# instadeepai/InstaGeo-E2E-Geospatial-ML

Hardware: AMD Instinct MI355X
Metric: HLS chips/sec (train fwd+bwd+AdamW), prithvi_eo_v1_100 224x224x6 T=1 (higher is better)
Workload: dtype bf16; 1 GPU; BASELINE.json configs[1]: Prithvi-100M fine-tune, Sen1Floods11-shaped synthetic int16 chips (6 bands, T=1, 224x224, 2 classes, weights [1,3], ignore -1, dropout 0.1); per_gpu_batch=432, global_batch=432, parallelism=dp1, launch=eager, deterministic=True

## Files before the change

instageo-e2e-geospatial-ml_amd/csrc/attention2.hip:

```cpp
#include <stdlib.h>

#include "common.h"

#ifdef IG_A2_PROF
__device__ unsigned long long g_a2prof[8 * 48];
#define A2P_INIT_X const bool a2p_on = blockIdx.x == 0 && blockIdx.y == 1 && blockIdx.z == 1 && (threadIdx.x & 63) == 0;
#define A2P_MARK(I) { if (a2p_on) g_a2prof[(threadIdx.x >> 6) * 48 + (I)] = __builtin_readcyclecounter(); }
#define A2P_MARKV(I, V) { float a2p_v = (V); asm volatile("" ::"v"(a2p_v)); if (a2p_on) g_a2prof[(threadIdx.x >> 6) * 48 + (I)] = __builtin_readcyclecounter(); }
extern "C" int ig_debug_a2prof(unsigned long long* dst) { return hipMemcpyFromSymbol(dst, HIP_SYMBOL(g_a2prof), sizeof(g_a2prof)) == hipSuccess ? 0 : -1; }
#else
#define A2P_INIT_X
#define A2P_MARK(I)
#define A2P_MARKV(I, V)
#endif

namespace {

constexpr int A2_WAVES = 7, A2_THREADS = 448, A2_QB = 224, A2_CH = 224;
constexpr int A2_TILE = A2_CH * 128;
typedef __attribute__((ext_vector_type(16))) float f32x16;
typedef __attribute__((ext_vector_type(8))) short s16x8;
typedef __attribute__((address_space(3))) s16x4* lds_s16x4;
typedef __attribute__((address_space(3))) char* lds_char_ptr;

__device__ __forceinline__ void glds16(const void* gsrc, unsigned lds_dst) {
    unsigned keep;
    lds_dst = __builtin_amdgcn_readfirstlane(lds_dst);
    asm volatile("s_mov_b32 %0, m0\n\ts_mov_b32 m0, %2\n\ts_nop 0\n\tglobal_load_lds_dwordx4 %1, off\n\ts_mov_b32 m0, %0"
                 : "=&s"(keep)
                 : "v"(gsrc), "s"(lds_dst)
                 : "memory");
}
__device__ __forceinline__ int k_swz(int row) { return (row >> 1) & 7; }
__device__ __forceinline__ int v_swz(int row) { return ((row >> 1) & 1) << 2; }

__device__ __forceinline__ f32x16 mfma32(bf16x8_t a, bf16x8_t b, f32x16 c) { return __builtin_amdgcn_mfma_f32_32x32x16_bf16(a, b, c, 0, 0, 0); }
template <bool SPLIT>
__device__ __forceinline__ f32x16 mma3(bf16x8_t ah, bf16x8_t al, bf16x8_t bh, bf16x8_t bl, f32x16 c) {
    c = mfma32(ah, bh, c);
    if constexpr (SPLIT) {
        c = mfma32(ah, bl, c);
        c = mfma32(al, bh, c);
    }
    return c;
}

template <bool SPLIT>
__device__ __forceinline__ void a2_store_row64(bf16_t* hi, bf16_t* lo, size_t orow, const f32x16 (&acc)[2], float scale, int lh) {
#pragma unroll
    for (int dh = 0; dh < 2; ++dh)
#pragma unroll
        for (int gp = 0; gp < 2; ++gp) {
            float va[4], vc[4];
#pragma unroll
            for (int e = 0; e < 4; ++e) va[e] = acc[dh][8 * gp + e] * scale, vc[e] = acc[dh][8 * gp + 4 + e] * scale;
            const uint32_t a0 = pack_bf2(va[0], va[1]), a1 = pack_bf2(va[2], va[3]), c0 = pack_bf2(vc[0], vc[1]), c1 = pack_bf2(vc[2], vc[3]);
            {
                const auto s0 = __builtin_amdgcn_permlane32_swap(a0, c0, false, false);
                const auto s1 = __builtin_amdgcn_permlane32_swap(a1, c1, false, false);
                *reinterpret_cast<uint4*>(hi + orow + 32 * dh + 16 * gp + 8 * lh) = lh == 0 ? make_uint4(a0, a1, s0[1], s1[1]) : make_uint4(s0[0], s1[0], c0, c1);
            }
            if constexpr (SPLIT) {
                const uint32_t la0 = pack_bf2(va[0] - __uint_as_float(a0 << 16), va[1] - __uint_as_float(a0 & 0xffff0000u));
                const uint32_t la1 = pack_bf2(va[2] - __uint_as_float(a1 << 16), va[3] - __uint_as_float(a1 & 0xffff0000u));
                const uint32_t lc0 = pack_bf2(vc[0] - __uint_as_float(c0 << 16), vc[1] - __uint_as_float(c0 & 0xffff0000u));
                const uint32_t lc1 = pack_bf2(vc[2] - __uint_as_float(c1 << 16), vc[3] - __uint_as_float(c1 & 0xffff0000u));
                const auto s0 = __builtin_amdgcn_permlane32_swap(la0, lc0, false, false);
                const auto s1 = __builtin_amdgcn_permlane32_swap(la1, lc1, false, false);
                *reinterpret_cast<uint4*>(lo + orow + 32 * dh + 16 * gp + 8 * lh) = lh == 0 ? make_uint4(la0, la1, s0[1], s1[1]) : make_uint4(s0[0], s1[0], lc0, lc1);
            }
        }
}

template <bool SPLIT>
__global__ __launch_bounds__(A2_THREADS) void attn2_fwd_kernel(const bf16_t* __restrict__ qkv_hi, const bf16_t* __restrict__ qkv_lo,
                                                               bf16_t* __restrict__ out_hi, bf16_t* __restrict__ out_lo,
                                                               float* __restrict__ lse, int N, int H, float scale) {
    extern __shared__ __attribute__((aligned(16))) char smem[];
    char* k_hi = smem;
    char* v_hi = smem + A2_TILE;
    char* k_lo = smem + 2 * A2_TILE;
    char* v_lo = smem + 3 * A2_TILE;
    const int tid = threadIdx.x, lane = tid & 63;
    const int wave = __builtin_amdgcn_readfirstlane(tid >> 6);
    const int lr = lane & 31, lh = lane >> 5;
    const int h = blockIdx.y, b = blockIdx.z;
    const long RS = 3L * H * 64;
    const bf16_t* base_hi = qkv_hi + (long)b * N * RS + h * 64;
    const bf16_t* base_lo = SPLIT ? qkv_lo + (long)b * N * RS + h * 64 : nullptr;
    const int q0 = blockIdx.x * A2_QB + wave * 32;
    const bool active = q0 < N;

    bf16x8_t qh[4], ql[4];
    {
        const int qr = min(q0 + lr, N - 1);
#pragma unroll
        for (int s = 0; s < 4; ++s) {
            qh[s] = __builtin_bit_cast(bf16x8_t, *reinterpret_cast<const uint4*>(base_hi + (long)qr * RS + 16 * s + 8 * lh));
            if constexpr (SPLIT) ql[s] = __builtin_bit_cast(bf16x8_t, *reinterpret_cast<const uint4*>(base_lo + (long)qr * RS + 16 * s + 8 * lh));
            else ql[s] = qh[s];
        }
    }
    f32x16 o[2];
#pragma unroll
    for (int i = 0; i < 2; ++i)
#pragma unroll
        for (int r = 0; r < 16; ++r) o[i][r] = 0.f;
    float m_run = -INFINITY, l_run = 0.f;
    const float c2 = scale * 1.44269504088896340736f;
    const unsigned lds_base = (unsigned)(uintptr_t)(lds_char_ptr)smem;

    for (int c0 = 0; c0 < N; c0 += A2_CH) {
        if (c0 > 0) __syncthreads();
#pragma unroll
        for (int i = 0; i < 4; ++i) {
            const int row = (wave * 4 + i) * 8 + (lane >> 3);
            const int key = min(c0 + row, N - 1);
            const long goff = (long)key * RS;
            const int ck = ((lane & 7) ^ k_swz(row)) * 8, cv = ((lane & 7) ^ v_swz(row)) * 8;
            const unsigned dst = lds_base + (wave * 4 + i) * 1024;
            glds16(base_hi + goff + H * 64 + ck, dst);
            glds16(base_hi + goff + 2 * H * 64 + cv, dst + A2_TILE);
            if constexpr (SPLIT) {
                glds16(base_lo + goff + H * 64 + ck, dst + 2 * A2_TILE);
                glds16(base_lo + goff + 2 * H * 64 + cv, dst + 3 * A2_TILE);
            }
        }
        asm volatile("s_waitcnt vmcnt(0)" ::: "memory");
        __syncthreads();
        if (!active) continue;
        const int ntile = min(A2_CH / 32, (N - c0 + 31) >> 5);
#define A2_QK(KT, DST)                                                                                       \
    {                                                                                                        \
        _Pragma("unroll") for (int r_ = 0; r_ < 16; ++r_) DST[r_] = 0.f;                                     \
        const int krow_ = (KT)*32 + lr;                                                                      \
        _Pragma("unroll") for (int s_ = 0; s_ < 4; ++s_) {                                                   \
            const int off_ = krow_ * 128 + (((2 * s_ + lh) ^ k_swz(krow_)) << 4);                            \
            const bf16x8_t kh_ = *reinterpret_cast<const bf16x8_t*>(k_hi + off_);                            \
            const bf16x8_t kl_ = SPLIT ? *reinterpret_cast<const bf16x8_t*>(k_lo + off_) : kh_;              \
            DST = mma3<SPLIT>(kh_, kl_, qh[s_], ql[s_], DST);                                                \
        }                                                                                                    \
    }
        f32x16 st_next;
        A2_QK(0, st_next)
        for (int kt = 0; kt < ntile; ++kt) {
            f32x16 st = st_next;
            if (kt + 1 < ntile) A2_QK(kt + 1, st_next)
            const int key0 = c0 + kt * 32;
            if (key0 + 32 > N) {
                asm volatile("" ::: "memory");
#pragma unroll
                for (int r = 0; r < 16; ++r)
                    if (key0 + 8 * (r >> 2) + 4 * lh + (r & 3) >= N) st[r] = -INFINITY;
            }
            float mx = st[0];
#pragma unroll
            for (int r = 1; r < 16; ++r) mx = fmaxf(mx, st[r]);
            {
                const auto sw = __builtin_amdgcn_permlane32_swap(__float_as_uint(mx), __float_as_uint(mx), false, false);
                mx = fmaxf(__uint_as_float(sw[0]), __uint_as_float(sw[1]));
            }
            const float m_tile = mx * c2;
            if (__builtin_amdgcn_ballot_w64(m_tile > m_run + 8.0f) != 0) {
                const float m_new = fmaxf(m_run, m_tile);
                const float alpha = __builtin_amdgcn_exp2f(m_run - m_new);
#pragma unroll
                for (int i = 0; i < 2; ++i)
// ... 234 lines not shown
#pragma unroll
        for (int o = 16; o >= 1; o >>= 1) {
            const bool up = (lr & o) != 0;
#pragma unroll
            for (int i = 0; i < o; ++i) {
                const float snd = up ? v[i] : v[i + o], kp = up ? v[i + o] : v[i];
                v[i] = kp + __shfl_xor(snd, o, 64);
            }
        }
        scr[(wave * 2 + 0) * 64 + 32 * (lr >> 4) + 8 * ((lr >> 2) & 3) + 4 * lh + (lr & 3)] = v[0];
    }
    {
        float v[32];
#pragma unroll
        for (int s = 0; s < 4; ++s)
#pragma unroll
            for (int e = 0; e < 8; ++e) {
                const float dv = SPLIT ? (float)dh[s][e] + (float)dl[s][e] : (float)dh[s][e];
                v[s * 8 + e] = valid ? dv : 0.f;
            }
#pragma unroll
        for (int o = 16; o >= 1; o >>= 1) {
            const bool up = (lr & o) != 0;
#pragma unroll
            for (int i = 0; i < o; ++i) {
                const float snd = up ? v[i] : v[i + o], kp = up ? v[i + o] : v[i];
                v[i] = kp + __shfl_xor(snd, o, 64);
            }
        }
        scr[(wave * 2 + 1) * 64 + 16 * (lr >> 3) + 8 * lh + (lr & 7)] = v[0];
    }
    __syncthreads();
    if (tid < 128) {
        const int part = tid >> 6, col = tid & 63;
        float t = 0.f;
#pragma unroll
        for (int w = 0; w < A2_WAVES; ++w) t += scr[(w * 2 + part) * 64 + col];
        ig_red_add(dbias + (size_t)(part * 2) * H * 64 + h * 64 + col, t);
    }
}

template <bool SPLIT>
__global__ __launch_bounds__(A2_THREADS) void attn2_bwd_dkv_kernel(const bf16_t* __restrict__ qkv_hi, const bf16_t* __restrict__ qkv_lo,
                                                                   const bf16_t* __restrict__ do_hi, const bf16_t* __restrict__ do_lo,
                                                                   const float* __restrict__ lse, const float* __restrict__ delta,
                                                                   bf16_t* __restrict__ dqkv_hi, bf16_t* __restrict__ dqkv_lo, int N, int H,
                                                                   float scale) {
    extern __shared__ __attribute__((aligned(16))) char smem[];
    char* q_hi = smem;
    char* d_hi = smem + A2_TILE;
    char* q_lo = smem + 2 * A2_TILE;
    char* d_lo = smem + 3 * A2_TILE;
    float* s_lse = reinterpret_cast<float*>(smem + (SPLIT ? 4 : 2) * A2_TILE);
    float* s_del = s_lse + A2_CH;
    const int tid = threadIdx.x, lane = tid & 63;
    const int wave = __builtin_amdgcn_readfirstlane(tid >> 6);
    const int lr = lane & 31, lh = lane >> 5;
    const int h = blockIdx.y, b = blockIdx.z;
    const long RS = 3L * H * 64, OS = (long)H * 64;
    const bf16_t* base_hi = qkv_hi + (long)b * N * RS + h * 64;
    const bf16_t* base_lo = SPLIT ? qkv_lo + (long)b * N * RS + h * 64 : nullptr;
    const bf16_t* dob_hi = do_hi + (long)b * N * OS + h * 64;
    const bf16_t* dob_lo = SPLIT ? do_lo + (long)b * N * OS + h * 64 : nullptr;
    const int k0 = blockIdx.x * A2_QB + wave * 32;
    const bool active = k0 < N;
    const int key = k0 + lr, kr = min(key, N - 1);

    bf16x8_t kh[4], kl[4], vh[4], vl[4];
#pragma unroll
    for (int s = 0; s < 4; ++s) {
        kh[s] = own_frag(base_hi + H * 64, RS, kr, s, lh);
        vh[s] = own_frag(base_hi + 2 * H * 64, RS, kr, s, lh);
        kl[s] = SPLIT ? own_frag(base_lo + H * 64, RS, kr, s, lh) : kh[s];
        vl[s] = SPLIT ? own_frag(base_lo + 2 * H * 64, RS, kr, s, lh) : vh[s];
    }
    const float c2 = scale * 1.44269504088896340736f;
    f32x16 dk[2], dv[2];
#pragma unroll
    for (int i = 0; i < 2; ++i)
#pragma unroll
        for (int r = 0; r < 16; ++r) dk[i][r] = 0.f, dv[i][r] = 0.f;
    const unsigned lds_base = (unsigned)(uintptr_t)(lds_char_ptr)smem;

    for (int c0 = 0; c0 < N; c0 += A2_CH) {
        if (c0 > 0) __syncthreads();
        dma_image(lds_base, base_hi, RS, c0, N, wave, lane);
        dma_image(lds_base + A2_TILE, dob_hi, OS, c0, N, wave, lane);
        if constexpr (SPLIT) {
            dma_image(lds_base + 2 * A2_TILE, base_lo, RS, c0, N, wave, lane);
            dma_image(lds_base + 3 * A2_TILE, dob_lo, OS, c0, N, wave, lane);
        }
        if (tid < A2_CH) {
            const int qq = c0 + tid;
            s_lse[tid] = qq < N ? lse[((long)b * H + h) * N + qq] * 1.44269504088896340736f : INFINITY;
            s_del[tid] = qq < N ? delta[((long)b * H + h) * N + qq] : 0.f;
        }
        asm volatile("s_waitcnt vmcnt(0)" ::: "memory");
        __syncthreads();
        if (!active) continue;
        const int ntile = min(A2_CH / 32, (N - c0 + 31) >> 5);
        for (int qt = 0; qt < ntile; ++qt) {
            f32x16 st, dp;
#pragma unroll
            for (int r = 0; r < 16; ++r) st[r] = 0.f, dp[r] = 0.f;
#pragma unroll
            for (int s = 0; s < 4; ++s) {
                const bf16x8_t ah = rows_frag(q_hi, qt * 32, s, lr, lh);
                const bf16x8_t al = SPLIT ? rows_frag(q_lo, qt * 32, s, lr, lh) : ah;
                st = mma3<SPLIT>(ah, al, kh[s], kl[s], st);
            }
#pragma unroll
            for (int s = 0; s < 4; ++s) {
                const bf16x8_t ah = rows_frag(d_hi, qt * 32, s, lr, lh);
                const bf16x8_t al = SPLIT ? rows_frag(d_lo, qt * 32, s, lr, lh) : ah;
                dp = mma3<SPLIT>(ah, al, vh[s], vl[s], dp);
            }
            f32x16 ds;
#pragma unroll
            for (int g = 0; g < 4; ++g) {
                const float4 l4 = *reinterpret_cast<const float4*>(s_lse + qt * 32 + 8 * g + 4 * lh);
                const float4 d4 = *reinterpret_cast<const float4*>(s_del + qt * 32 + 8 * g + 4 * lh);
                const float ll[4] = {l4.x, l4.y, l4.z, l4.w}, dd[4] = {d4.x, d4.y, d4.z, d4.w};
#pragma unroll
                for (int e = 0; e < 4; ++e) {
                    const float pv = __builtin_amdgcn_exp2f(fmaf(st[4 * g + e], c2, -ll[e]));
                    st[4 * g + e] = pv;
                    ds[4 * g + e] = pv * (dp[4 * g + e] - dd[e]);
                }
            }
#pragma unroll
            for (int s = 0; s < 2; ++s) {
                bf16x8_t ph, pl, sh, sl;
                pack_step<SPLIT>(st, s, ph, pl);
                pack_step<SPLIT>(ds, s, sh, sl);
#pragma unroll
                for (int dhf = 0; dhf < 2; ++dhf) {
                    const bf16x8_t th = tr_frag(d_hi, qt * 32, s, 32 * dhf, lane);
                    const bf16x8_t tl = SPLIT ? tr_frag(d_lo, qt * 32, s, 32 * dhf, lane) : th;
                    dv[dhf] = mma3<SPLIT>(th, tl, ph, pl, dv[dhf]);
                    const bf16x8_t uh = tr_frag(q_hi, qt * 32, s, 32 * dhf, lane);
                    const bf16x8_t ul = SPLIT ? tr_frag(q_lo, qt * 32, s, 32 * dhf, lane) : uh;
                    dk[dhf] = mma3<SPLIT>(uh, ul, sh, sl, dk[dhf]);
                }
            }
        }
    }
    if (!active || key >= N) return;
    const size_t orow = ((size_t)b * N + key) * RS + h * 64;
    a2_store_row64<SPLIT>(dqkv_hi, dqkv_lo, orow + (size_t)H * 64, dk, scale, lh);
    a2_store_row64<SPLIT>(dqkv_hi, dqkv_lo, orow + 2 * (size_t)H * 64, dv, 1.f, lh);
}


constexpr int A2F_DQP = 68;
constexpr int A2F_SLAB = 32 * 72;
constexpr int A2F_OFF_K = 2 * A2_TILE;
constexpr int A2F_OFF_DQ = 2 * A2_TILE;
constexpr int A2F_OFF_SLAB = A2F_OFF_DQ + A2_CH * A2F_DQP * 4;
constexpr int A2F_OFF_LSE = A2F_OFF_SLAB + A2_WAVES * A2F_SLAB;
constexpr int A2F_SMEM = A2F_OFF_LSE + 2 * A2_CH * 4;

__device__ __forceinline__ bf16x8_t tr_slab(const char* slab, int s, int lane) {
    const int g16 = lane >> 4, i16 = lane & 15;
    const int r0 = 16 * s + 4 * (g16 >> 1) + (i16 >> 2), r1 = r0 + 8;
    const int cb = (16 * (g16 & 1) + 4 * (i16 & 3)) * 2;
    const s16x4 a0 = __builtin_amdgcn_ds_read_tr16_b64_v4i16((lds_s16x4)(slab + r0 * 72 + cb));
    const s16x4 a1 = __builtin_amdgcn_ds_read_tr16_b64_v4i16((lds_s16x4)(slab + r1 * 72 + cb));
    const s16x8 av = {a0[0], a0[1], a0[2], a0[3], a1[0], a1[1], a1[2], a1[3]};
    return __builtin_bit_cast(bf16x8_t, av);
}

__global__ __launch_bounds__(A2_THREADS) void attn2_bwd_fused_kernel(const bf16_t* __restrict__ qkv_hi, const bf16_t* __restrict__ do_hi,
                                                                     const bf16_t* __restrict__ o_hi, const float* __restrict__ lse,
                                                                     float* __restrict__ delta, bf16_t* __restrict__ dqkv_hi, int N, int H,
                                                                     float scale, float* __restrict__ dbias) {
    extern __shared__ __attribute__((aligned(16))) char smem[];
    A2P_INIT_X
    char* q_img = smem;
    char* d_img = smem + A2_TILE;
    char* k_img = smem + A2F_OFF_K;
    float* s_dq = reinterpret_cast<float*>(smem + A2F_OFF_DQ);
    float* s_lse = reinterpret_cast<float*>(smem + A2F_OFF_LSE);
    float* s_del = s_lse + A2_CH;
    const int tid = threadIdx.x, lane = tid & 63;
    const int wave = __builtin_amdgcn_readfirstlane(tid >> 6);
    char* slab = smem + A2F_OFF_SLAB + wave * A2F_SLAB;
    const int lr = lane & 31, lh = lane >> 5;
    const long RS = 3L * H * 64, OS = (long)H * 64;
    const int h = blockIdx.y, b = blockIdx.z;
    const bf16_t* base = qkv_hi + (long)b * N * RS + h * 64;
    const bf16_t* dob = do_hi + (long)b * N * OS + h * 64;
    const bf16_t* ob = o_hi + (long)b * N * OS + h * 64;
    const int k0 = wave * 32;
    const bool active = k0 < N;
    const int key = k0 + lr, kr = min(key, N - 1);
    const unsigned lds_base = (unsigned)(uintptr_t)(lds_char_ptr)smem;

    dma_image(lds_base, base, RS, 0, N, wave, lane);
    dma_image(lds_base + A2_TILE, dob, OS, 0, N, wave, lane);
    dma_image(lds_base + A2F_OFF_K, base + H * 64, RS, 0, N, wave, lane);
    bf16x8_t kh[4], vh[4];
#pragma unroll
    for (int s = 0; s < 4; ++s) {
        kh[s] = own_frag(base + H * 64, RS, kr, s, lh);
        vh[s] = own_frag(base + 2 * H * 64, RS, kr, s, lh);
    }
    {
        float dl = 0.f;
#pragma unroll
        for (int s = 0; s < 4; ++s) {
            const bf16x8_t oh = own_frag(ob, OS, kr, s, lh), dh = own_frag(dob, OS, kr, s, lh);
#pragma unroll
            for (int e = 0; e < 8; ++e) dl = fmaf((float)oh[e], (float)dh[e], dl);
        }
        const auto sw = __builtin_amdgcn_permlane32_swap(__float_as_uint(dl), __float_as_uint(dl), false, false);
        dl = __uint_as_float(sw[0]) + __uint_as_float(sw[1]);
        if (lh == 0) {
            if (key < N) delta[((long)b * H + h) * N + key] = dl;
            s_lse[key] = key < N ? lse[((long)b * H + h) * N + key] * 1.44269504088896340736f : INFINITY;
            s_del[key] = key < N ? dl : 0.f;
        }
    }
    const float c2 = scale * 1.44269504088896340736f;
    const float kmask = key < N ? 1.f : 0.f;
    f32x16 dk[2], dv[2];
#pragma unroll
    for (int i = 0; i < 2; ++i)
#pragma unroll
        for (int r = 0; r < 16; ++r) dk[i][r] = 0.f, dv[i][r] = 0.f;
    A2P_MARK(0)
    asm volatile("s_waitcnt vmcnt(0)" ::: "memory");
    A2P_MARK(1)
    __syncthreads();
    A2P_MARK(2)
    const int ntile = (N + 31) >> 5;
    bf16x8_t kt[2][2];
#pragma unroll
    for (int s = 0; s < 2; ++s)
#pragma unroll
        for (int dhf = 0; dhf < 2; ++dhf) kt[s][dhf] = tr_frag(k_img, k0, s, 32 * dhf, lane);
    asm volatile("s_waitcnt lgkmcnt(0)" ::: "memory");
    __syncthreads();
    A2P_MARK(3)
    for (int step = 0; step < A2_WAVES; ++step) {
        const int qt = (wave + step) % A2_WAVES;
        A2P_MARK(4 + step * 6)
        if (active && qt < ntile) {
            f32x16 st, dp;
#pragma unroll
            for (int r = 0; r < 16; ++r) st[r] = 0.f, dp[r] = 0.f;
#pragma unroll
            for (int s = 0; s < 4; ++s) st = mfma32(rows_frag(q_img, qt * 32, s, lr, lh), kh[s], st);
#pragma unroll
            for (int s = 0; s < 4; ++s) dp = mfma32(rows_frag(d_img, qt * 32, s, lr, lh), vh[s], dp);
            bf16x8_t tdo[2][2], tq[2][2];
#pragma unroll
            for (int s = 0; s < 2; ++s)
#pragma unroll
                for (int dhf = 0; dhf < 2; ++dhf) {
                    tdo[s][dhf] = tr_frag(d_img, qt * 32, s, 32 * dhf, lane);
                    tq[s][dhf] = tr_frag(q_img, qt * 32, s, 32 * dhf, lane);
                }
            A2P_MARKV(5 + step * 6, st[0] + dp[0])
            f32x16 ds;
#pragma unroll
            for (int g = 0; g < 4; ++g) {
                const float4 l4 = *reinterpret_cast<const float4*>(s_lse + qt * 32 + 8 * g + 4 * lh);
                const float4 d4 = *reinterpret_cast<const float4*>(s_del + qt * 32 + 8 * g + 4 * lh);
                const float ll[4] = {l4.x, l4.y, l4.z, l4.w}, dd[4] = {d4.x, d4.y, d4.z, d4.w};
#pragma unroll
                for (int e = 0; e < 4; ++e) {
                    const float pv = __builtin_amdgcn_exp2f(fmaf(st[4 * g + e], c2, -ll[e])) * kmask;
                    st[4 * g + e] = pv;
                    ds[4 * g + e] = pv * (dp[4 * g + e] - dd[e]);
                }
            }
            A2P_MARKV(6 + step * 6, ds[0] + ds[15])
#pragma unroll
            for (int s = 0; s < 2; ++s) {
                bf16x8_t ph, pl, sh, sl;
                pack_step<false>(st, s, ph, pl);
                pack_step<false>(ds, s, sh, sl);
                const uint4 su = __builtin_bit_cast(uint4, sh);
                *reinterpret_cast<uint2*>(slab + lr * 72 + (16 * s + 4 * lh) * 2) = make_uint2(su.x, su.y);
                *reinterpret_cast<uint2*>(slab + lr * 72 + (16 * s + 8 + 4 * lh) * 2) = make_uint2(su.z, su.w);
#pragma unroll
                for (int dhf = 0; dhf < 2; ++dhf) {
                    dv[dhf] = mfma32(tdo[s][dhf], ph, dv[dhf]);
                    dk[dhf] = mfma32(tq[s][dhf], sh, dk[dhf]);
                }
            }
            A2P_MARKV(7 + step * 6, dv[0][0] + dk[0][0] + dv[1][15] + dk[1][15])
            asm volatile("s_waitcnt lgkmcnt(0)" ::: "memory");
            f32x16 dq0, dq1;
            {
                const float* row = s_dq + (qt * 32 + lr) * A2F_DQP + 4 * lh;
#pragma unroll
                for (int g = 0; g < 4; ++g) {
                    float4 o0 = make_float4(0.f, 0.f, 0.f, 0.f), o1 = o0;
                    if (step > 0) o0 = *reinterpret_cast<const float4*>(row + 8 * g), o1 = *reinterpret_cast<const float4*>(row + 32 + 8 * g);
                    dq0[4 * g] = o0.x, dq0[4 * g + 1] = o0.y, dq0[4 * g + 2] = o0.z, dq0[4 * g + 3] = o0.w;
                    dq1[4 * g] = o1.x, dq1[4 * g + 1] = o1.y, dq1[4 * g + 2] = o1.z, dq1[4 * g + 3] = o1.w;
                }
            }
            const bf16x8_t b0 = tr_slab(slab, 0, lane), b1 = tr_slab(slab, 1, lane);
            dq0 = mfma32(kt[0][0], b0, dq0);
            dq1 = mfma32(kt[0][1], b0, dq1);
            dq0 = mfma32(kt[1][0], b1, dq0);
            dq1 = mfma32(kt[1][1], b1, dq1);
            {
                float* row = s_dq + (qt * 32 + lr) * A2F_DQP + 4 * lh;
#pragma unroll
                for (int g = 0; g < 4; ++g) {
                    *reinterpret_cast<float4*>(row + 8 * g) = make_float4(dq0[4 * g], dq0[4 * g + 1], dq0[4 * g + 2], dq0[4 * g + 3]);
                    *reinterpret_cast<float4*>(row + 32 + 8 * g) = make_float4(dq1[4 * g], dq1[4 * g + 1], dq1[4 * g + 2], dq1[4 * g + 3]);
                }
            }
            A2P_MARK(8 + step * 6)
        }
        __syncthreads();
        A2P_MARK(9 + step * 6)
    }
    float cbq[8] = {0.f, 0.f, 0.f, 0.f, 0.f, 0.f, 0.f, 0.f}, cbv[8] = {0.f, 0.f, 0.f, 0.f, 0.f, 0.f, 0.f, 0.f};
    for (int it = tid; it < N * 8; it += A2_THREADS) {
        const int q = it >> 3, c = it & 7;
        const float4 v0 = *reinterpret_cast<const float4*>(s_dq + q * A2F_DQP + 8 * c), v1 = *reinterpret_cast<const float4*>(s_dq + q * A2F_DQP + 8 * c + 4);
        const float f[8] = {v0.x * scale, v0.y * scale, v0.z * scale, v0.w * scale, v1.x * scale, v1.y * scale, v1.z * scale, v1.w * scale};
        *reinterpret_cast<uint4*>(dqkv_hi + ((size_t)b * N + q) * RS + h * 64 + 8 * c) = pack8(f);
#pragma unroll
        for (int e = 0; e < 8; ++e) cbq[e] += f[e];
    }
    A2P_MARK(46)
    if (dbias) {
        for (int it = tid; it < N * 8; it += A2_THREADS) {
            const int q = it >> 3, c = it & 7;
            float f[8];
            unpack8(*reinterpret_cast<const uint4*>(d_img + q * 128 + ((c ^ sw2(q)) << 4)), f);
#pragma unroll
            for (int e = 0; e < 8; ++e) cbv[e] += f[e];
        }
        A2P_MARKV(40, cbv[0] + cbv[7])
        float* scr = reinterpret_cast<float*>(q_img);
        *reinterpret_cast<float4*>(scr + tid * 16) = make_float4(cbq[0], cbq[1], cbq[2], cbq[3]);
        *reinterpret_cast<float4*>(scr + tid * 16 + 4) = make_float4(cbq[4], cbq[5], cbq[6], cbq[7]);
        *reinterpret_cast<float4*>(scr + tid * 16 + 8) = make_float4(cbv[0], cbv[1], cbv[2], cbv[3]);
        *reinterpret_cast<float4*>(scr + tid * 16 + 12) = make_float4(cbv[4], cbv[5], cbv[6], cbv[7]);
        A2P_MARK(41)
        __syncthreads();
        A2P_MARK(42)
        if (tid < 128) {
            const int part = tid >> 6, col = tid & 63;
            float t = 0.f;
            for (int g = 0; g < A2_THREADS / 8; ++g) t += scr[(g * 8 + (col >> 3)) * 16 + part * 8 + (col & 7)];
            ig_red_add(dbias + (size_t)(part * 2) * H * 64 + h * 64 + col, t);
        }
    }
    A2P_MARK(47)
    if (active && key < N) {
        const size_t orow = ((size_t)b * N + key) * RS + h * 64;
        a2_store_row64<false>(dqkv_hi, nullptr, orow + (size_t)H * 64, dk, scale, lh);
        a2_store_row64<false>(dqkv_hi, nullptr, orow + 2 * (size_t)H * 64, dv, 1.f, lh);
    }
}

}
IG_DET_TU(attention2)

int ig_attention2_fwd(const void* qkv_hi, const void* qkv_lo, void* out_hi, void* out_lo, float* lse, int B, int N, int H, void* stream) {
    IG_REQUIRE(N >= 1 && H <= 65535 && B <= 65535, "ig_attention_fwd: B and H must be <= 65535 (grid dimensions), got B = %d, H = %d", B, H);
    IG_REQUIRE((((uintptr_t)qkv_hi | (uintptr_t)qkv_lo) & 15) == 0, "ig_attention_fwd: qkv must be 16-byte aligned%s", "");
    const bool split = qkv_lo != nullptr;
    const dim3 grid((N + A2_QB - 1) / A2_QB, H, B);
    const int lds = (split ? 4 : 2) * A2_TILE;
    const float scale = 0.125f;
    hipStream_t st = (hipStream_t)stream;
    if (split) {
        static bool attr = false;
        if (!attr) {
            (void)hipFuncSetAttribute((const void*)attn2_fwd_kernel<true>, hipFuncAttributeMaxDynamicSharedMemorySize, lds);
            attr = true;
        }
        ig_note_kernel("attn2_fwd_kernel<true>");
        hipLaunchKernelGGL(attn2_fwd_kernel<true>, grid, dim3(A2_THREADS), lds, st, (const bf16_t*)qkv_hi, (const bf16_t*)qkv_lo,
                           (bf16_t*)out_hi, (bf16_t*)out_lo, lse, N, H, scale);
    } else {
        static bool attr = false;
        if (!attr) {
            (void)hipFuncSetAttribute((const void*)attn2_fwd_kernel<false>, hipFuncAttributeMaxDynamicSharedMemorySize, lds);
            attr = true;
        }
        ig_note_kernel("attn2_fwd_kernel<false>");
        hipLaunchKernelGGL(attn2_fwd_kernel<false>, grid, dim3(A2_THREADS), lds, st, (const bf16_t*)qkv_hi, (const bf16_t*)qkv_lo,
                           (bf16_t*)out_hi, (bf16_t*)out_lo, lse, N, H, scale);
    }
    return ig_check_launch("ig_attention_fwd(attn2)");
}

int ig_attention2_bwd(const void* qkv_hi, const void* qkv_lo, const void* out_hi, const void* out_lo, const void* dout_hi,
                      const void* dout_lo, const float* lse, float* delta, void* dqkv_hi, void* dqkv_lo, float* dbias, int B, int N, int H,
                      void* stream) {
    IG_REQUIRE(N >= 1 && H <= 65535 && B <= 65535, "ig_attention_bwd: B and H must be <= 65535 (grid dimensions), got B = %d, H = %d", B, H);
    IG_REQUIRE((((uintptr_t)qkv_hi | (uintptr_t)qkv_lo | (uintptr_t)dout_hi | (uintptr_t)dout_lo | (uintptr_t)out_hi | (uintptr_t)out_lo) & 15) == 0,
               "ig_attention_bwd: the tensors must be 16-byte aligned%s", "");
    const bool split = qkv_lo != nullptr;
    const dim3 grid((N + A2_QB - 1) / A2_QB, H, B);
    const int lds_q = (split ? 4 : 2) * A2_TILE, lds_kv = lds_q + 2 * A2_CH * (int)sizeof(float);
    const float scale = 0.125f;
    hipStream_t st = (hipStream_t)stream;
    if (!split && N <= A2_CH) {
        static bool attr = false;
        if (!attr) {
            (void)hipFuncSetAttribute((const void*)attn2_bwd_fused_kernel, hipFuncAttributeMaxDynamicSharedMemorySize, A2F_SMEM);
            attr = true;
        }
        ig_note_kernel("attn2_bwd_fused_kernel");
        hipLaunchKernelGGL(attn2_bwd_fused_kernel, dim3(1, H, B), dim3(A2_THREADS), A2F_SMEM, st, (const bf16_t*)qkv_hi, (const bf16_t*)dout_hi,
                           (const bf16_t*)out_hi, lse, delta, (bf16_t*)dqkv_hi, N, H, scale, dbias);
        return ig_check_launch("ig_attention_bwd(attn2 fused)");
    }
    constexpr int dqlb = 4;
    float* dbias_k = dbias;
#define IG_A2_BWD(SPLIT_)                                                                                                          \
    {                                                                                                                              \
        static bool attr = false;                                                                                                  \
        if (!attr) {                                                                                                               \
            (void)hipFuncSetAttribute((const void*)attn2_bwd_dq_kernel<SPLIT_, 2>, hipFuncAttributeMaxDynamicSharedMemorySize, lds_q); \
            (void)hipFuncSetAttribute((const void*)attn2_bwd_dq_kernel<SPLIT_, 4>, hipFuncAttributeMaxDynamicSharedMemorySize, lds_q); \
            (void)hipFuncSetAttribute((const void*)attn2_bwd_dkv_kernel<SPLIT_>, hipFuncAttributeMaxDynamicSharedMemorySize, lds_kv); \
            attr = true;                                                                                                           \
        }                                                                                                                          \
        if (dqlb == 4 && !SPLIT_)                                                                                                  \
            hipLaunchKernelGGL((attn2_bwd_dq_kernel<SPLIT_, 4>), grid, dim3(A2_THREADS), lds_q, st, (const bf16_t*)qkv_hi,          \
                               (const bf16_t*)qkv_lo, (const bf16_t*)dout_hi, (const bf16_t*)dout_lo, (const bf16_t*)out_hi,       \
                               (const bf16_t*)out_lo, lse, delta, (bf16_t*)dqkv_hi, (bf16_t*)dqkv_lo, N, H, scale, dbias_k);       \
        else                                                                                                                       \
            hipLaunchKernelGGL((attn2_bwd_dq_kernel<SPLIT_, 2>), grid, dim3(A2_THREADS), lds_q, st, (const bf16_t*)qkv_hi,          \
                               (const bf16_t*)qkv_lo, (const bf16_t*)dout_hi, (const bf16_t*)dout_lo, (const bf16_t*)out_hi,       \
                               (const bf16_t*)out_lo, lse, delta, (bf16_t*)dqkv_hi, (bf16_t*)dqkv_lo, N, H, scale, dbias_k);       \
        ig_note_kernel("attn2_bwd_dq_kernel<%s>+attn2_bwd_dkv_kernel<%s>", SPLIT_ ? "true" : "false", SPLIT_ ? "true" : "false");  \
        hipLaunchKernelGGL(attn2_bwd_dkv_kernel<SPLIT_>, grid, dim3(A2_THREADS), lds_kv, st, (const bf16_t*)qkv_hi,                   \
                           (const bf16_t*)qkv_lo, (const bf16_t*)dout_hi, (const bf16_t*)dout_lo, lse, delta, (bf16_t*)dqkv_hi,     \
                           (bf16_t*)dqkv_lo, N, H, scale);                                                                         \
    }
    if (split) IG_A2_BWD(true) else IG_A2_BWD(false)
#undef IG_A2_BWD
    return ig_check_launch("ig_attention_bwd(attn2)");
}
```

Before: 5424 chips/s.

## Replace fused attention backward with two-phase 4-wave kernel fitting two workgroups per CU

```diff
diff --git a/instageo-e2e-geospatial-ml_amd/csrc/attention2.hip b/instageo-e2e-geospatial-ml_amd/csrc/attention2.hip
--- a/instageo-e2e-geospatial-ml_amd/csrc/attention2.hip
+++ b/instageo-e2e-geospatial-ml_amd/csrc/attention2.hip
@@ -1,18 +1,6 @@
 #include <stdlib.h>
 
 #include "common.h"
-
-#ifdef IG_A2_PROF
-__device__ unsigned long long g_a2prof[8 * 48];
-#define A2P_INIT_X const bool a2p_on = blockIdx.x == 0 && blockIdx.y == 1 && blockIdx.z == 1 && (threadIdx.x & 63) == 0;
-#define A2P_MARK(I) { if (a2p_on) g_a2prof[(threadIdx.x >> 6) * 48 + (I)] = __builtin_readcyclecounter(); }
-#define A2P_MARKV(I, V) { float a2p_v = (V); asm volatile("" ::"v"(a2p_v)); if (a2p_on) g_a2prof[(threadIdx.x >> 6) * 48 + (I)] = __builtin_readcyclecounter(); }
-extern "C" int ig_debug_a2prof(unsigned long long* dst) { return hipMemcpyFromSymbol(dst, HIP_SYMBOL(g_a2prof), sizeof(g_a2prof)) == hipSuccess ? 0 : -1; }
-#else
-#define A2P_INIT_X
-#define A2P_MARK(I)
-#define A2P_MARKV(I, V)
-#endif
 
 namespace {
 
@@ -553,116 +541,97 @@
 }
 
 
-constexpr int A2F_DQP = 68;
-constexpr int A2F_SLAB = 32 * 72;
-constexpr int A2F_OFF_K = 2 * A2_TILE;
-constexpr int A2F_OFF_DQ = 2 * A2_TILE;
-constexpr int A2F_OFF_SLAB = A2F_OFF_DQ + A2_CH * A2F_DQP * 4;
-constexpr int A2F_OFF_LSE = A2F_OFF_SLAB + A2_WAVES * A2F_SLAB;
-constexpr int A2F_SMEM = A2F_OFF_LSE + 2 * A2_CH * 4;
-
-__device__ __forceinline__ bf16x8_t tr_slab(const char* slab, int s, int lane) {
-    const int g16 = lane >> 4, i16 = lane & 15;
-    const int r0 = 16 * s + 4 * (g16 >> 1) + (i16 >> 2), r1 = r0 + 8;
-    const int cb = (16 * (g16 & 1) + 4 * (i16 & 3)) * 2;
-    const s16x4 a0 = __builtin_amdgcn_ds_read_tr16_b64_v4i16((lds_s16x4)(slab + r0 * 72 + cb));
-    const s16x4 a1 = __builtin_amdgcn_ds_read_tr16_b64_v4i16((lds_s16x4)(slab + r1 * 72 + cb));
-    const s16x8 av = {a0[0], a0[1], a0[2], a0[3], a1[0], a1[1], a1[2], a1[3]};
-    return __builtin_bit_cast(bf16x8_t, av);
-}
-
-__global__ __launch_bounds__(A2_THREADS) void attn2_bwd_fused_kernel(const bf16_t* __restrict__ qkv_hi, const bf16_t* __restrict__ do_hi,
-                                                                     const bf16_t* __restrict__ o_hi, const float* __restrict__ lse,
-                                                                     float* __restrict__ delta, bf16_t* __restrict__ dqkv_hi, int N, int H,
-                                                                     float scale, float* __restrict__ dbias) {
-    extern __shared__ __attribute__((aligned(16))) char smem[];
-    A2P_INIT_X
-    char* q_img = smem;
-    char* d_img = smem + A2_TILE;
-    char* k_img = smem + A2F_OFF_K;
-    float* s_dq = reinterpret_cast<float*>(smem + A2F_OFF_DQ);
-    float* s_lse = reinterpret_cast<float*>(smem + A2F_OFF_LSE);
+constexpr int A2O_WAVES = 4, A2O_THREADS = 256;
+constexpr int A2O_OFF_LSE = 2 * A2_TILE;
+constexpr int A2O_SMEM = A2O_OFF_LSE + 2 * A2_CH * 4;
+static_assert(2 * A2O_SMEM <= 160 * 1024, "two workgroups of the single-pass backward must fit the 160 KB of LDS of a CU");
+
+__device__ __forceinline__ void dma_image4(unsigned lds_img, const bf16_t* gbase, long rs, int ngrp, int N, int wave, int lane) {
+    for (int g = wave; g < ngrp; g += A2O_WAVES) {
+        const int row = g * 8 + (lane >> 3);
+        const int tok = min(row, N - 1);
+        glds16(gbase + (long)tok * rs + (((lane & 7) ^ sw2(row)) * 8), lds_img + g * 1024);
+    }
+}
+
+__global__ __launch_bounds__(A2O_THREADS, 2) void attn2_bwd_onepass_kernel(const bf16_t* __restrict__ qkv_hi, const bf16_t* __restrict__ do_hi,
+                                                                           const bf16_t* __restrict__ o_hi, const float* __restrict__ lse,
+                                                                           float* __restrict__ delta, bf16_t* __restrict__ dqkv_hi, int N, int H,
+                                                                           float scale, float* __restrict__ dbias) {
+    __shared__ __attribute__((aligned(16))) char smem[A2O_SMEM];
+    char* img0 = smem;
+    char* img1 = smem + A2_TILE;
+    float* s_lse = reinterpret_cast<float*>(smem + A2O_OFF_LSE);
     float* s_del = s_lse + A2_CH;
     const int tid = threadIdx.x, lane = tid & 63;
     const int wave = __builtin_amdgcn_readfirstlane(tid >> 6);
-    char* slab = smem + A2F_OFF_SLAB + wave * A2F_SLAB;
     const int lr = lane & 31, lh = lane >> 5;
     const long RS = 3L * H * 64, OS = (long)H * 64;
     const int h = blockIdx.y, b = blockIdx.z;
     const bf16_t* base = qkv_hi + (long)b * N * RS + h * 64;
     const bf16_t* dob = do_hi + (long)b * N * OS + h * 64;
     const bf16_t* ob = o_hi + (long)b * N * OS + h * 64;
-    const int k0 = wave * 32;
-    const bool active = k0 < N;
-    const int key = k0 + lr, kr = min(key, N - 1);
+    const long lrow = ((long)b * H + h) * N;
+    const int ntile = (N + 31) >> 5;
     const unsigned lds_base = (unsigned)(uintptr_t)(lds_char_ptr)smem;
-
-    dma_image(lds_base, base, RS, 0, N, wave, lane);
-    dma_image(lds_base + A2_TILE, dob, OS, 0, N, wave, lane);
-    dma_image(lds_base + A2F_OFF_K, base + H * 64, RS, 0, N, wave, lane);
-    bf16x8_t kh[4], vh[4];
-#pragma unroll
-    for (int s = 0; s < 4; ++s) {
-        kh[s] = own_frag(base + H * 64, RS, kr, s, lh);
-        vh[s] = own_frag(base + 2 * H * 64, RS, kr, s, lh);
-    }
-    {
+    const float c2 = scale * 1.44269504088896340736f;
+
+    dma_image4(lds_base, base, RS, ntile * 4, N, wave, lane);
+    dma_image4(lds_base + A2_TILE, dob, OS, ntile * 4, N, wave, lane);
+    for (int t = wave; t < ntile; t += A2O_WAVES) {
+        const int q = t * 32 + lr, qr = min(q, N - 1);
         float dl = 0.f;
 #pragma unroll
         for (int s = 0; s < 4; ++s) {
-            const bf16x8_t oh = own_frag(ob, OS, kr, s, lh), dh = own_frag(dob, OS, kr, s, lh);
+            const bf16x8_t oh = own_frag(ob, OS, qr, s, lh), dh = own_frag(dob, OS, qr, s, lh);
 #pragma unroll
             for (int e = 0; e < 8; ++e) dl = fmaf((float)oh[e], (float)dh[e], dl);
         }
         const auto sw = __builtin_amdgcn_permlane32_swap(__float_as_uint(dl), __float_as_uint(dl), false, false);
         dl = __uint_as_float(sw[0]) + __uint_as_float(sw[1]);
         if (lh == 0) {
-            if (key < N) delta[((long)b * H + h) * N + key] = dl;
-            s_lse[key] = key < N ? lse[((long)b * H + h) * N + key] * 1.44269504088896340736f : INFINITY;
-            s_del[key] = key < N ? dl : 0.f;
-        }
-    }
-    const float c2 = scale * 1.44269504088896340736f;
-    const float kmask = key < N ? 1.f : 0.f;
-    f32x16 dk[2], dv[2];
-#pragma unroll
-    for (int i = 0; i < 2; ++i)
-#pragma unroll
-        for (int r = 0; r < 16; ++r) dk[i][r] = 0.f, dv[i][r] = 0.f;
-    A2P_MARK(0)
+            if (q < N) delta[lrow + q] = dl;
+            s_lse[q] = q < N ? lse[lrow + q] * 1.44269504088896340736f : INFINITY;
+            s_del[q] = q < N ? dl : 0.f;
+        }
+    }
+    bf16x8_t kh[4], vh[4];
+    auto load_kv = [&](int kt) {
+        const int kr = min(kt * 32 + lr, N - 1);
+#pragma unroll
+        for (int s = 0; s < 4; ++s) {
+            kh[s] = own_frag(base + H * 64, RS, kr, s, lh);
+            vh[s] = own_frag(base + 2 * H * 64, RS, kr, s, lh);
+        }
+    };
+    if (wave < ntile) load_kv(wave);
     asm volatile("s_waitcnt vmcnt(0)" ::: "memory");
-    A2P_MARK(1)
     __syncthreads();
-    A2P_MARK(2)
-    const int ntile = (N + 31) >> 5;
-    bf16x8_t kt[2][2];
-#pragma unroll
-    for (int s = 0; s < 2; ++s)
-#pragma unroll
-        for (int dhf = 0; dhf < 2; ++dhf) kt[s][dhf] = tr_frag(k_img, k0, s, 32 * dhf, lane);
-    asm volatile("s_waitcnt lgkmcnt(0)" ::: "memory");
-    __syncthreads();
-    A2P_MARK(3)
-    for (int step = 0; step < A2_WAVES; ++step) {
-        const int qt = (wave + step) % A2_WAVES;
-        A2P_MARK(4 + step * 6)
-        if (active && qt < ntile) {
+
+    for (int kt = wave; kt < ntile; kt += A2O_WAVES) {
+        const int key = kt * 32 + lr;
+        if (kt != wave) load_kv(kt);
+        f32x16 dk[2], dv[2];
+#pragma unroll
+        for (int i = 0; i < 2; ++i)
+#pragma unroll
+            for (int r = 0; r < 16; ++r) dk[i][r] = 0.f, dv[i][r] = 0.f;
+        for (int qt = 0; qt < ntile; ++qt) {
             f32x16 st, dp;
 #pragma unroll
             for (int r = 0; r < 16; ++r) st[r] = 0.f, dp[r] = 0.f;
 #pragma unroll
-            for (int s = 0; s < 4; ++s) st = mfma32(rows_frag(q_img, qt * 32, s, lr, lh), kh[s], st);
-#pragma unroll
-            for (int s = 0; s < 4; ++s) dp = mfma32(rows_frag(d_img, qt * 32, s, lr, lh), vh[s], dp);
+            for (int s = 0; s < 4; ++s) st = mfma32(rows_frag(img0, qt * 32, s, lr, lh), kh[s], st);
+#pragma unroll
+            for (int s = 0; s < 4; ++s) dp = mfma32(rows_frag(img1, qt * 32, s, lr, lh), vh[s], dp);
             bf16x8_t tdo[2][2], tq[2][2];
 #pragma unroll
             for (int s = 0; s < 2; ++s)
 #pragma unroll
                 for (int dhf = 0; dhf < 2; ++dhf) {
-                    tdo[s][dhf] = tr_frag(d_img, qt * 32, s, 32 * dhf, lane);
-                    tq[s][dhf] = tr_frag(q_img, qt * 32, s, 32 * dhf, lane);
+                    tdo[s][dhf] = tr_frag(img1, qt * 32, s, 32 * dhf, lane);
+                    tq[s][dhf] = tr_frag(img0, qt * 32, s, 32 * dhf, lane);
                 }
-            A2P_MARKV(5 + step * 6, st[0] + dp[0])
             f32x16 ds;
 #pragma unroll
             for (int g = 0; g < 4; ++g) {
@@ -671,96 +640,122 @@
                 const float ll[4] = {l4.x, l4.y, l4.z, l4.w}, dd[4] = {d4.x, d4.y, d4.z, d4.w};
 #pragma unroll
                 for (int e = 0; e < 4; ++e) {
-                    const float pv = __builtin_amdgcn_exp2f(fmaf(st[4 * g + e], c2, -ll[e])) * kmask;
+                    const float pv = __builtin_amdgcn_exp2f(fmaf(st[4 * g + e], c2, -ll[e]));
                     st[4 * g + e] = pv;
                     ds[4 * g + e] = pv * (dp[4 * g + e] - dd[e]);
                 }
             }
-            A2P_MARKV(6 + step * 6, ds[0] + ds[15])
 #pragma unroll
             for (int s = 0; s < 2; ++s) {
                 bf16x8_t ph, pl, sh, sl;
                 pack_step<false>(st, s, ph, pl);
                 pack_step<false>(ds, s, sh, sl);
-                const uint4 su = __builtin_bit_cast(uint4, sh);
-                *reinterpret_cast<uint2*>(slab + lr * 72 + (16 * s + 4 * lh) * 2) = make_uint2(su.x, su.y);
-                *reinterpret_cast<uint2*>(slab + lr * 72 + (16 * s + 8 + 4 * lh) * 2) = make_uint2(su.z, su.w);
 #pragma unroll
                 for (int dhf = 0; dhf < 2; ++dhf) {
                     dv[dhf] = mfma32(tdo[s][dhf], ph, dv[dhf]);
                     dk[dhf] = mfma32(tq[s][dhf], sh, dk[dhf]);
                 }
             }
-            A2P_MARKV(7 + step * 6, dv[0][0] + dk[0][0] + dv[1][15] + dk[1][15])
-            asm volatile("s_waitcnt lgkmcnt(0)" ::: "memory");
-            f32x16 dq0, dq1;
-            {
-                const float* row = s_dq + (qt * 32 + lr) * A2F_DQP + 4 * lh;
-#pragma unroll
-                for (int g = 0; g < 4; ++g) {
-                    float4 o0 = make_float4(0.f, 0.f, 0.f, 0.f), o1 = o0;
-                    if (step > 0) o0 = *reinterpret_cast<const float4*>(row + 8 * g), o1 = *reinterpret_cast<const float4*>(row + 32 + 8 * g);
-                    dq0[4 * g] = o0.x, dq0[4 * g + 1] = o0.y, dq0[4 * g + 2] = o0.z, dq0[4 * g + 3] = o0.w;
-                    dq1[4 * g] = o1.x, dq1[4 * g + 1] = o1.y, dq1[4 * g + 2] = o1.z, dq1[4 * g + 3] = o1.w;
-                }
-            }
-            const bf16x8_t b0 = tr_slab(slab, 0, lane), b1 = tr_slab(slab, 1, lane);
-            dq0 = mfma32(kt[0][0], b0, dq0);
-            dq1 = mfma32(kt[0][1], b0, dq1);
-            dq0 = mfma32(kt[1][0], b1, dq0);
-            dq1 = mfma32(kt[1][1], b1, dq1);
-            {
-                float* row = s_dq + (qt * 32 + lr) * A2F_DQP + 4 * lh;
-#pragma unroll
-                for (int g = 0; g < 4; ++g) {
-                    *reinterpret_cast<float4*>(row + 8 * g) = make_float4(dq0[4 * g], dq0[4 * g + 1], dq0[4 * g + 2], dq0[4 * g + 3]);
-                    *reinterpret_cast<float4*>(row + 32 + 8 * g) = make_float4(dq1[4 * g], dq1[4 * g + 1], dq1[4 * g + 2], dq1[4 * g + 3]);
-                }
-            }
-            A2P_MARK(8 + step * 6)
-        }
-        __syncthreads();
-        A2P_MARK(9 + step * 6)
-    }
-    float cbq[8] = {0.f, 0.f, 0.f, 0.f, 0.f, 0.f, 0.f, 0.f}, cbv[8] = {0.f, 0.f, 0.f, 0.f, 0.f, 0.f, 0.f, 0.f};
-    for (int it = tid; it < N * 8; it += A2_THREADS) {
-        const int q = it >> 3, c = it & 7;
-        const float4 v0 = *reinterpret_cast<const float4*>(s_dq + q * A2F_DQP + 8 * c), v1 = *reinterpret_cast<const float4*>(s_dq + q * A2F_DQP + 8 * c + 4);
-        const float f[8] = {v0.x * scale, v0.y * scale, v0.z * scale, v0.w * scale, v1.x * scale, v1.y * scale, v1.z * scale, v1.w * scale};
-        *reinterpret_cast<uint4*>(dqkv_hi + ((size_t)b * N + q) * RS + h * 64 + 8 * c) = pack8(f);
-#pragma unroll
-        for (int e = 0; e < 8; ++e) cbq[e] += f[e];
-    }
-    A2P_MARK(46)
-    if (dbias) {
-        for (int it = tid; it < N * 8; it += A2_THREADS) {
-            const int q = it >> 3, c = it & 7;
-            float f[8];
-            unpack8(*reinterpret_cast<const uint4*>(d_img + q * 128 + ((c ^ sw2(q)) << 4)), f);
-#pragma unroll
-            for (int e = 0; e < 8; ++e) cbv[e] += f[e];
-        }
-        A2P_MARKV(40, cbv[0] + cbv[7])
-        float* scr = reinterpret_cast<float*>(q_img);
-        *reinterpret_cast<float4*>(scr + tid * 16) = make_float4(cbq[0], cbq[1], cbq[2], cbq[3]);
-        *reinterpret_cast<float4*>(scr + tid * 16 + 4) = make_float4(cbq[4], cbq[5], cbq[6], cbq[7]);
-        *reinterpret_cast<float4*>(scr + tid * 16 + 8) = make_float4(cbv[0], cbv[1], cbv[2], cbv[3]);
-        *reinterpret_cast<float4*>(scr + tid * 16 + 12) = make_float4(cbv[4], cbv[5], cbv[6], cbv[7]);
-        A2P_MARK(41)
-        __syncthreads();
-        A2P_MARK(42)
-        if (tid < 128) {
-            const int part = tid >> 6, col = tid & 63;
-            float t = 0.f;
-            for (int g = 0; g < A2_THREADS / 8; ++g) t += scr[(g * 8 + (col >> 3)) * 16 + part * 8 + (col & 7)];
-            ig_red_add(dbias + (size_t)(part * 2) * H * 64 + h * 64 + col, t);
-        }
-    }
-    A2P_MARK(47)
-    if (active && key < N) {
-        const size_t orow = ((size_t)b * N + key) * RS + h * 64;
-        a2_store_row64<false>(dqkv_hi, nullptr, orow + (size_t)H * 64, dk, scale, lh);
-        a2_store_row64<false>(dqkv_hi, nullptr, orow + 2 * (size_t)H * 64, dv, 1.f, lh);
+        }
+        if (key < N) {
+            const size_t orow = ((size_t)b * N + key) * RS + h * 64;
+            a2_store_row64<false>(dqkv_hi, nullptr, orow + (size_t)H * 64, dk, scale, lh);
+            a2_store_row64<false>(dqkv_hi, nullptr, orow + 2 * (size_t)H * 64, dv, 1.f, lh);
+        }
+    }
+
+    __syncthreads();
+    dma_image4(lds_base, base + H * 64, RS, ntile * 4, N, wave, lane);
+    dma_image4(lds_base + A2_TILE, base + 2 * H * 64, RS, ntile * 4, N, wave, lane);
+    bf16x8_t qh[4], dh[4];
+    auto load_qdo = [&](int qt) {
+        const int qr = min(qt * 32 + lr, N - 1);
+#pragma unroll
+        for (int s = 0; s < 4; ++s) {
+            qh[s] = own_frag(base, RS, qr, s, lh);
+            dh[s] = own_frag(dob, OS, qr, s, lh);
+        }
+    };
+    if (wave < ntile) load_qdo(wave);
+    asm volatile("s_waitcnt vmcnt(0)" ::: "memory");
+    __syncthreads();
+    float cq[32], cv[32];
+#pragma unroll
+    for (int i = 0; i < 32; ++i) cq[i] = 0.f, cv[i] = 0.f;
+    for (int qt = wave; qt < ntile; qt += A2O_WAVES) {
+        const int q = qt * 32 + lr;
+        if (qt != wave) load_qdo(qt);
+        const float my_lse = s_lse[q], my_delta = s_del[q];
+        f32x16 dq[2];
+#pragma unroll
+        for (int i = 0; i < 2; ++i)
+#pragma unroll
+            for (int r = 0; r < 16; ++r) dq[i][r] = 0.f;
+        for (int kt = 0; kt < ntile; ++kt) {
+            f32x16 st, dp;
+#pragma unroll
+            for (int r = 0; r < 16; ++r) st[r] = 0.f, dp[r] = 0.f;
+#pragma unroll
+            for (int s = 0; s < 4; ++s) st = mfma32(rows_frag(img0, kt * 32, s, lr, lh), qh[s], st);
+#pragma unroll
+            for (int s = 0; s < 4; ++s) dp = mfma32(rows_frag(img1, kt * 32, s, lr, lh), dh[s], dp);
+            bf16x8_t tk[2][2];
+#pragma unroll
+            for (int s = 0; s < 2; ++s)
+#pragma unroll
+                for (int dhf = 0; dhf < 2; ++dhf) tk[s][dhf] = tr_frag(img0, kt * 32, s, 32 * dhf, lane);
+            const int key0 = kt * 32;
+            if (key0 + 32 > N) {
+                asm volatile("" ::: "memory");
+#pragma unroll
+                for (int r = 0; r < 16; ++r)
+                    if (key0 + 8 * (r >> 2) + 4 * lh + (r & 3) >= N) st[r] = -INFINITY;
+            }
+#pragma unroll
+            for (int r = 0; r < 16; ++r)
+                st[r] = __builtin_amdgcn_exp2f(fmaf(st[r], c2, -my_lse)) * (dp[r] - my_delta);
+#pragma unroll
+            for (int s = 0; s < 2; ++s) {
+                bf16x8_t sh, sl;
+                pack_step<false>(st, s, sh, sl);
+#pragma unroll
+                for (int dhf = 0; dhf < 2; ++dhf) dq[dhf] = mfma32(tk[s][dhf], sh, dq[dhf]);
+            }
+        }
+        const bool valid = q < N;
+        if (valid) a2_store_row64<false>(dqkv_hi, nullptr, ((size_t)b * N + q) * RS + h * 64, dq, scale, lh);
+        if (dbias) {
+#pragma unroll
+            for (int i = 0; i < 32; ++i) cq[i] += valid ? dq[i >> 4][i & 15] * scale : 0.f;
+#pragma unroll
+            for (int s = 0; s < 4; ++s)
+#pragma unroll
+                for (int e = 0; e < 8; ++e) cv[8 * s + e] += valid ? (float)dh[s][e] : 0.f;
+        }
+    }
+    if (!dbias) return;
+    __syncthreads();
+    float* scr = reinterpret_cast<float*>(smem);
+#pragma unroll
+    for (int o = 16; o >= 1; o >>= 1) {
+        const bool up = (lr & o) != 0;
+#pragma unroll
+        for (int i = 0; i < o; ++i) {
+            const float snd = up ? cq[i] : cq[i + o], kp = up ? cq[i + o] : cq[i];
+            cq[i] = kp + __shfl_xor(snd, o, 64);
+            const float snd2 = up ? cv[i] : cv[i + o], kp2 = up ? cv[i + o] : cv[i];
+            cv[i] = kp2 + __shfl_xor(snd2, o, 64);
+        }
+    }
+    scr[(wave * 2 + 0) * 64 + 32 * (lr >> 4) + 8 * ((lr >> 2) & 3) + 4 * lh + (lr & 3)] = cq[0];
+    scr[(wave * 2 + 1) * 64 + 16 * (lr >> 3) + 8 * lh + (lr & 7)] = cv[0];
+    __syncthreads();
+    if (tid < 128) {
+        const int part = tid >> 6, col = tid & 63;
+        float t = 0.f;
+#pragma unroll
+        for (int w = 0; w < A2O_WAVES; ++w) t += scr[(w * 2 + part) * 64 + col];
+        ig_red_add(dbias + (size_t)(part * 2) * H * 64 + h * 64 + col, t);
     }
 }
 
@@ -809,15 +804,10 @@
     const float scale = 0.125f;
     hipStream_t st = (hipStream_t)stream;
     if (!split && N <= A2_CH) {
-        static bool attr = false;
-        if (!attr) {
-            (void)hipFuncSetAttribute((const void*)attn2_bwd_fused_kernel, hipFuncAttributeMaxDynamicSharedMemorySize, A2F_SMEM);
-            attr = true;
-        }
-        ig_note_kernel("attn2_bwd_fused_kernel");
-        hipLaunchKernelGGL(attn2_bwd_fused_kernel, dim3(1, H, B), dim3(A2_THREADS), A2F_SMEM, st, (const bf16_t*)qkv_hi, (const bf16_t*)dout_hi,
+        ig_note_kernel("attn2_bwd_onepass_kernel");
+        hipLaunchKernelGGL(attn2_bwd_onepass_kernel, dim3(1, H, B), dim3(A2O_THREADS), 0, st, (const bf16_t*)qkv_hi, (const bf16_t*)dout_hi,
                            (const bf16_t*)out_hi, lse, delta, (bf16_t*)dqkv_hi, N, H, scale, dbias);
-        return ig_check_launch("ig_attention_bwd(attn2 fused)");
+        return ig_check_launch("ig_attention_bwd(attn2 onepass)");
     }
     constexpr int dqlb = 4;
     float* dbias_k = dbias;
```

Measured after the change: 5482 chips/s, median of 6. 1.01x the previous value.
